# caojiezhang/CiaoSR

Measured on AMD Instinct MI355X. Metric: HR Mpix/s (RDN-CiaoSR x4, LocalImplicitSR forward_test), higher is better.
Workload: dtype f32; 1 GPU; C3: RDN-CiaoSR (c64b16) x4, LR 1356x2040 -> 5424x8160 (DIV2K-shaped 2K LR), tiled inference: 117 tiles of 192x192 (overlap 32), random-init weights, fp32; scale=4, tiles=117, parallelism=tile-shard x1

## Files before the change

### ciaosr_amd/csrc/csa_scores_f32.hip

```cpp
#include "ops.h"

namespace ciaosr {

typedef float f32x16 __attribute__((ext_vector_type(16)));
typedef int i32x4 __attribute__((ext_vector_type(4)));

constexpr int BSH = 8, BSW = 16;
constexpr int BLH = 4, BLW = 16;
constexpr int BHW = BSW + 2;
constexpr int BPN = (BSH + 2) * BHW;
constexpr int BLN = (BLH + 2) * BHW;
constexpr int BDP = 109;
constexpr int BDB = BPN * BDP * 4;
constexpr size_t kBoxLds = 2 * (size_t)BDB;
constexpr unsigned kOobB = 0xFFFFFFF0u;

struct BoxP {
    const float* M; int ldm; unsigned m_bytes; int Hp, Wp;
    int y0, y1;
    const float* R; int ldr; unsigned r_bytes; int Hl, Wl;
    const float* nrm;
    float* S; int lds_; size_t s_floats;
    int pbx, lbx, n_lb, n_items;
};

__global__ void csa_key_norms_kernel(const float* __restrict__ R, int ldr, int Hl, int Wl, int Ch, float floor_, float alpha,
                                     float* __restrict__ nrm) {
    const int lane = threadIdx.x & 63;
    const long l = (long)blockIdx.x * 4 + (threadIdx.x >> 6);
    if (l >= (long)Hl * Wl) return;
    const int ly = (int)(l / Wl), lx = (int)(l - (long)ly * Wl);
    float ss = 0.f;
    for (int e = lane; e < 9 * Ch; e += 64) {
        const int tap = e / Ch, c = e - tap * Ch;
        const int y = ly + tap / 3 - 1, x = lx + tap % 3 - 1;
        if (y >= 0 && y < Hl && x >= 0 && x < Wl) {
            const float v = R[((size_t)y * Wl + x) * ldr + c];
            ss += v * v;
        }
    }
#pragma unroll
    for (int o = 32; o > 0; o >>= 1) ss += __shfl_xor(ss, o, 64);
    if (lane == 0) nrm[l] = alpha / fmaxf(sqrtf(ss), floor_);
}

__global__ __launch_bounds__(512) void csa_scores_box_f32_kernel(BoxP p) {
    extern __shared__ __attribute__((aligned(16))) float Dl[];
    const int t = threadIdx.x, lane = t & 63, wv = __builtin_amdgcn_readfirstlane(t >> 6), li = lane & 31, lh = lane >> 5;
    const int per = (p.n_items + (int)gridDim.x - 1) / (int)gridDim.x;
    const int i0 = (int)blockIdx.x * per, i1 = min(i0 + per, p.n_items);
    if (i0 >= i1) return;
    auto item_pb = [&](int it) -> int { return it / p.n_lb; };
    auto item_lb = [&](int it) -> int { return it - (it / p.n_lb) * p.n_lb; };

    if (wv < 4) {
        const __amdgpu_buffer_rsrc_t rs_m = __builtin_amdgcn_make_buffer_rsrc(const_cast<float*>(p.M), 0, p.m_bytes, 0x00020000);
        const __amdgpu_buffer_rsrc_t rs_r = __builtin_amdgcn_make_buffer_rsrc(const_cast<float*>(p.R), 0, p.r_bytes, 0x00020000);
        auto row_off = [&](int h, int hn, int y0, int x0, int Hh, int Ww, int ld) -> unsigned {
            const int hy = h / BHW, hx = h - hy * BHW;
            const int y = y0 - 1 + hy, x = x0 - 1 + hx;
            return (h < hn && y >= 0 && y < Hh && x >= 0 && x < Ww) ? (unsigned)(((size_t)y * Ww + x) * ld * 4) + (unsigned)lh * 16u : kOobB;
        };
        i32x4 fa[6][4];
        i32x4 fbc[4], fbn[4];
        auto load_a = [&](int pb) {
            const int py0 = p.y0 + (pb / p.pbx) * BSH, px0 = (pb % p.pbx) * BSW;
#pragma unroll
            for (int pt = 0; pt < 6; ++pt) {
                const unsigned mo = row_off(32 * pt + li, BPN, py0, px0, p.Hp, p.Wp, p.ldm);
#pragma unroll
                for (int j = 0; j < 4; ++j) fa[pt][j] = __builtin_amdgcn_raw_buffer_load_b128(rs_m, mo == kOobB ? (int)kOobB : (int)(mo + 32u * j), 0, 0);
            }
        };
        auto load_b = [&](int lb, i32x4 (&f)[4]) {
            const int ly0 = (lb / p.lbx) * BLH, lx0 = (lb % p.lbx) * BLW;
            const unsigned ro = row_off(32 * wv + li, BLN, ly0, lx0, p.Hl, p.Wl, p.ldr);
#pragma unroll
            for (int j = 0; j < 4; ++j) f[j] = __builtin_amdgcn_raw_buffer_load_b128(rs_r, ro == kOobB ? (int)kOobB : (int)(ro + 32u * j), 0, 0);
        };
        int cur_pb = item_pb(i0);
        load_a(cur_pb);
        load_b(item_lb(i0), fbc);
#pragma unroll 1
        for (int it = i0; it <= i1; ++it) {
            if (it < i1) {
                const int k = (it - i0) & 1;
                if (it + 1 < i1) load_b(item_lb(it + 1), fbn);
                float* D = Dl + k * (BDB / 4);
                const int lcol = 32 * wv + li;
#pragma unroll
                for (int pt = 0; pt < 6; ++pt) {
                    f32x16 acc;
#pragma unroll
                    for (int e = 0; e < 16; ++e) acc[e] = 0.f;
#pragma unroll
                    for (int j = 0; j < 4; ++j) {
                        const i32x4 a = fa[pt][j], b = fbc[j];
                        acc = __builtin_amdgcn_mfma_f32_32x32x2f32(__int_as_float(a.x), __int_as_float(b.x), acc, 0, 0, 0);
                        acc = __builtin_amdgcn_mfma_f32_32x32x2f32(__int_as_float(a.y), __int_as_float(b.y), acc, 0, 0, 0);
                        acc = __builtin_amdgcn_mfma_f32_32x32x2f32(__int_as_float(a.z), __int_as_float(b.z), acc, 0, 0, 0);
                        acc = __builtin_amdgcn_mfma_f32_32x32x2f32(__int_as_float(a.w), __int_as_float(b.w), acc, 0, 0, 0);
                    }
                    if (lcol < BLN) {
                        float* dcol = D + (4 * lh) * BDP + lcol;
#pragma unroll
                        for (int r = 0; r < 16; ++r) {
                            constexpr int kLast = BPN - 1;
                            const int rr = 32 * pt + (r & 3) + 8 * (r >> 2);
                            if (rr + 4 <= kLast) dcol[rr * BDP] = acc[r];
                            else if (rr <= kLast && lh == 0) dcol[rr * BDP] = acc[r];
                        }
                    }
                }
#pragma unroll
                for (int j = 0; j < 4; ++j) fbc[j] = fbn[j];
                if (it + 1 < i1 && item_pb(it + 1) != cur_pb) {
                    cur_pb = item_pb(it + 1);
                    load_a(cur_pb);
                }
            }
            __syncthreads();
        }
    } else {
        const int lyy = lane >> 4, lxx = lane & 15;
        int lcol9[9];
#pragma unroll
        for (int a = 0; a < 3; ++a)
#pragma unroll
            for (int b = 0; b < 3; ++b) lcol9[3 * a + b] = (lyy + a) * BHW + lxx + b;
        const int q0 = 32 * (wv - 4);
#pragma unroll 1
        for (int it = i0; it <= i1; ++it) {
            if (it > i0) {
                const int ci = it - 1, k = (ci - i0) & 1;
                const int pb = item_pb(ci), lb = item_lb(ci);
                const int py0 = p.y0 + (pb / p.pbx) * BSH, px0 = (pb % p.pbx) * BSW;
                const int ly = (lb / p.lbx) * BLH + lyy, lx = (lb % p.lbx) * BLW + lxx;
                const bool l_ok = ly < p.Hl && lx < p.Wl;
                const float sc = l_ok ? p.nrm[(size_t)ly * p.Wl + lx] : 0.f;
                const float* D = Dl + k * (BDB / 4) + (q0 >> 4) * BHW * BDP;
                const unsigned lane_off = l_ok ? (unsigned)((size_t)ly * p.Wl + lx) * 4u : kOobB;
                const int qy0 = py0 + (q0 >> 4);
                const size_t s_base = ((size_t)(qy0 - p.y0) * p.Wp + px0) * p.lds_;
                const size_t s_left = p.s_floats > s_base ? (p.s_floats - s_base) * 4 : 0;
                const size_t s_span = ((size_t)p.Wp + BSW) * p.lds_ * 4;
                const __amdgpu_buffer_rsrc_t rs_s =
                    __builtin_amdgcn_make_buffer_rsrc(p.S + s_base, 0, (unsigned)(s_left < s_span ? s_left : s_span), 0x00020000);
                const float* dk[9];
#pragma unroll
                for (int e = 0; e < 9; ++e) dk[e] = D + lcol9[e];
#pragma unroll
                for (int q = 0; q < 32; ++q) {
                    const int pyy = q >> 4, pxx = q & 15;
                    float s = dk[0][(pyy * BHW + pxx) * BDP];
#pragma unroll
                    for (int e = 1; e < 9; ++e) s += dk[e][((pyy + e / 3) * BHW + pxx + e % 3) * BDP];
                    const bool row_ok = qy0 + pyy < p.y1 && px0 + pxx < p.Wp;
                    const unsigned soff = (unsigned)(((size_t)pyy * p.Wp + pxx) * p.lds_ * 4);
                    __builtin_amdgcn_raw_buffer_store_b32(__float_as_int(s * sc), rs_s, (int)(row_ok ? lane_off : kOobB), (int)(row_ok ? soff : 0u), 0);
                }
            }
            __syncthreads();
        }
    }
}

bool csa_scores_box_ok(int Ch, int ldm, int ldr) { return Ch == 32 && (ldm & 3) == 0 && (ldr & 3) == 0; }

int csa_key_norms(const float* R, int ldr, int Hl, int Wl, int Ch, float alpha, float floor_, float* nrm, hipStream_t s) {
    CIAOSR_CHECK_ARG(R && nrm && csa_scores_box_ok(Ch, Ch, ldr));
    ProfScope prof("csa_key_norms", s);
    hipLaunchKernelGGL(csa_key_norms_kernel, dim3(ceil_div((long)Hl * Wl, 4)), dim3(256), 0, s, R, ldr, Hl, Wl, Ch, floor_, alpha, nrm);
    return launch_status("csa_key_norms");
}

int csa_scores_box_f32(const float* M, int ldm, int Hp, int Wp, const float* R, int ldr, int Hl, int Wl, int Ch, const float* nrm, float* S,
                       int ld_s, int y0, int y1, hipStream_t s) {
    CIAOSR_CHECK_ARG(M && R && nrm && S && csa_scores_box_ok(Ch, ldm, ldr) && aligned16(M) && aligned16(R) && 0 <= y0 && y0 < y1 && y1 <= Hp);
    const size_t mb = (size_t)Hp * Wp * ldm * 4, rb = (size_t)Hl * Wl * ldr * 4;
    const size_t s_floats = ((size_t)(y1 - y0) * Wp - 1) * ld_s + (size_t)Hl * Wl;
    CIAOSR_CHECK_ARG(mb < 0xFFFFFF00ull && rb < 0xFFFFFF00ull && ((size_t)Wp + BSW) * ld_s * 4 < 0xFFFFFF00ull);
    BoxP p;
    p.M = M; p.ldm = ldm; p.m_bytes = (unsigned)mb; p.Hp = Hp; p.Wp = Wp; p.y0 = y0; p.y1 = y1;
    p.R = R; p.ldr = ldr; p.r_bytes = (unsigned)rb; p.Hl = Hl; p.Wl = Wl;
    p.nrm = nrm; p.S = S; p.lds_ = ld_s; p.s_floats = s_floats;
    p.pbx = ceil_div(Wp, BSW); p.lbx = ceil_div(Wl, BLW);
    p.n_lb = ceil_div(Hl, BLH) * p.lbx;
    const long n_items = (long)ceil_div(y1 - y0, BSH) * p.pbx * p.n_lb;
    CIAOSR_CHECK_ARG(n_items < 0x7FFFFFFF);
    p.n_items = (int)n_items;
    CIAOSR_BIG_LDS(csa_scores_box_f32_kernel, kBoxLds);
    ProfScope prof("csa_scores", s);
    hipLaunchKernelGGL(csa_scores_box_f32_kernel, dim3(p.n_items < 256 ? p.n_items : 256), dim3(512), kBoxLds, s, p);
    return launch_status("csa_scores_box_f32");
}

}
```

### ciaosr_amd/csrc/csattn.hip

```cpp
#include "ops.h"

namespace ciaosr {

struct CsaPlan {
    int H, W, C, sc, Hp, Wp, HWp, Hl, Wl, L, Lld, Lld8, Ch;
    int band_rows, up, down, s_rows;
    size_t n_V, n_S, n_Y;
    bool banded() const { return band_rows < Hp; }
};

static CsaPlan csa_plan(int H, int W, int C, int sc) {
    CsaPlan p;
    p.H = H; p.W = W; p.C = C; p.sc = sc; p.Ch = (int)round_up(C / 2, 4);
    p.Hp = (int)round_up((size_t)H, sc); p.Wp = (int)round_up((size_t)W, sc);
    p.HWp = p.Hp * p.Wp; p.Hl = p.Hp / sc; p.Wl = p.Wp / sc; p.L = p.Hl * p.Wl;
    p.Lld = (int)round_up(p.L, 4); p.Lld8 = (int)round_up(p.L, 8);
    p.band_rows = p.s_rows = p.Hp; p.up = p.down = 0;
    p.n_V = (size_t)p.L * 9 * sc * sc * C; p.n_S = (size_t)p.HWp * p.Lld; p.n_Y = (size_t)sc * sc * p.HWp * C;
    return p;
}

static bool csa_composed(const CsaPlan& p, const ciaosr_options_t* opt) {
    const int composed_min = opt && opt->csa_composed_min ? opt->csa_composed_min : 4096;
    return p.sc == 2 && composed_min > 0 && p.HWp >= composed_min;
}
static bool csa_wants_four(const CsaPlan& p, Prec prec, const ciaosr_options_t* opt, int s_rows) {
    return prec == kF32 && !(opt && opt->csa_attn_v16) && csa_composed(p, opt) && csa_attn_v4_ok(p.Hp, p.Wp, p.C, p.Lld, s_rows);
}

constexpr int kCsaItemRows = 8;
constexpr int kCsaMinRows16 = 4;
static void csa_plan_bands(CsaPlan& p, Prec prec, const ciaosr_options_t* opt) {
    if (!opt || opt->csa_block_mb <= 0) return;
    const size_t budget = (size_t)opt->csa_block_mb << 20, row_s = (size_t)p.Wp * p.Lld * sizeof(float);
    const size_t row = row_s + (prec != kF32 ? (size_t)p.Wp * p.Lld8 * 2 : 0);
    if (budget >= row * p.Hp) return;
    const size_t min_rows = prec == kF32 ? kCsaItemRows : kCsaMinRows16;
    const bool four = csa_wants_four(p, prec, opt, kCsaItemRows);
    size_t sr = budget / row;
    const size_t addr = ((four ? 0x80000000ull : 0xFFFFFF00ull) - 1) / row_s;
    if (sr > addr) sr = addr;
    if (sr >= 2 * kCsaItemRows) sr -= sr % kCsaItemRows;
    if (sr < min_rows) sr = min_rows;
    const int halo = four ? 3 : 0;
    if (sr >= (size_t)p.Hp + halo) return;
    p.band_rows = (int)sr - halo; p.up = four ? 2 : 0; p.down = four ? 1 : 0;
    p.s_rows = (int)sr < p.Hp ? (int)sr : p.Hp;
    p.n_S = (size_t)p.s_rows * p.Wp * p.Lld;
}

struct CsaBuffers : CsaPlan {
    float *xp, *E, *M, *x2, *R, *Qp, *Kn, *V, *S, *O, *Y, *Yp, *PE, *Pc, *Vp, *Ov, *Er;
    unsigned short* P16;
    float* stats() const { return banded() ? V : Qp; }
    float* norms() const { return Kn; }
    float* partial4() const { return O; }
    float* vedge() const { return Vp; }
    float* edge_rows() const { return banded() ? Er : S; }
    float* splitk() const { return Y; }
    float* softmax_scratch() const { return S; }
    unsigned short* q16() const { return reinterpret_cast<unsigned short*>(Y); }
    unsigned short* k16() const { return q16() + round_up((size_t)HWp * 9 * Ch, 128); }
    unsigned short* vpT() const { return reinterpret_cast<unsigned short*>(V); }
    float* otop() const { return Ov; }
    float* oleft() const { return Ov + (size_t)Wp * 4 * C; }
    float* otl() const { return oleft() + (size_t)Hp * 4 * C; }
};
static bool qk16_fits(const CsaPlan& p) { return ((size_t)p.HWp + p.L) * 9 * p.Ch * 2 + 512 <= p.n_Y * sizeof(float); }
static bool vpt_fits(const CsaPlan& p) { return (size_t)25 * p.C * p.Lld8 * 2 <= p.n_V * sizeof(float); }
static bool softmax16_fits(const CsaPlan& p, const H16Ops& h) { return h.softmax_gemm_scratch((long)p.s_rows * p.Wp, p.L) <= p.n_S; }

template <class Take>
static CsaBuffers csa_carve(const CsaPlan& p, bool p16, Take take) {
    const size_t HW = p.HWp, L = p.L, C = p.C, Ch = p.Ch, n_PE = (size_t)(p.Hp / 2 + 3) * (p.Wp / 2 + 3) * 9 * C;
    CsaBuffers b = {p};
    b.xp = take(HW * C);
    b.E = take(HW * C); b.M = take(HW * Ch);
    b.x2 = take(L * C); b.R = take(L * Ch);
    b.Qp = take(HW * 9 * Ch); b.Kn = take(L * 9 * Ch);
    b.V = take(p.n_V);
    b.S = take(p.n_S);
    b.O = take(HW * 9 * p.sc * p.sc * C);
    b.Y = take(p.n_Y); b.Yp = take((size_t)p.H * p.W * 9 * C);
    b.PE = take(n_PE); b.Pc = take(n_PE);
    b.Vp = take(L * 25 * C);
    b.Ov = take((size_t)(p.Hp + p.Wp) * 4 * C + C);
    b.P16 = reinterpret_cast<unsigned short*>(take((p16 ? (size_t)p.s_rows * p.Wp * p.Lld8 / 2 : 0) + 64));
    b.Er = p.banded() ? take((size_t)(p.Wp + p.Hp) * p.Lld) : nullptr;
    return b;
}
static size_t csa_carve_bytes(const CsaPlan& p, bool p16) {
    size_t n = 0;
    csa_carve(p, p16, [&](size_t floats) { n += floats; return (float*)nullptr; });
    return n * sizeof(float) + 24 * 256;
}

enum CsaScores { kScoresBox, kScoresGemm, kScores16 };
enum CsaTail { kTailUncomposed, kTail16C, kTailFour, kTail16 };
struct CsaRoute {
    CsaScores scores; CsaTail tail;
    bool tile128;
    bool fused_softmax;
};

static CsaRoute csa_route(const CsaPlan& p, Prec prec, const ciaosr_options_t* opt, const ciaosr_csattn_weights_t* w) {
    CsaRoute r = {kScoresGemm, kTailUncomposed, opt && opt->csa_attn_tile128, false};
    if (prec == kF32 && !(opt && opt->csa_scores_gemm) && csa_scores_box_ok(p.Ch, p.Ch, p.Ch)) r.scores = kScoresBox;
    if (!(csa_composed(p, opt) && w->w_down_masked)) return r;
    if (prec != kF32 && (9 * p.Ch) % 8 == 0 && (p.Lld & 3) == 0 && qk16_fits(p) && vpt_fits(p)) {
        r.scores = kScores16; r.tail = kTail16;
        r.fused_softmax = softmax16_fits(p, h16_ops(prec)) && w->softmax_scale > 0.f;
    } else if (csa_wants_four(p, prec, opt, p.s_rows)) {
        r.tail = kTailFour;
    } else {
        r.tail = kTail16C;
    }
    return r;
}
static bool csa_attn_big(const CsaPlan& p, const CsaRoute& r, int M) {
    return !r.tile128 && gemm_big_softmax_f32_ok(p.Lld, 25 * p.C, M, 16 * p.C, p.L, true) &&
           ((size_t)(M - 1) * p.Lld + p.L) * sizeof(float) < 0xFFFFFF00ull;
}

struct CsaBand {
    int y0, y1, ya, yb;
    bool first() const { return y0 == 0; }
};

#define CSA_RUN(x) do { const int rc_ = (x); if (rc_ != CIAOSR_OK) return rc_; } while (0)
struct CsaCall : CsaBuffers {
    const ciaosr_csattn_weights_t* w; float* out; int ld_out; hipStream_t s;

    CsaBand band(int y0) const {
        const int y1 = y0 + band_rows < Hp ? y0 + band_rows : Hp;
        return {y0, y1, y0 > up ? y0 - up : 0, y1 + down < Hp ? y1 + down : Hp};
    }
    static int npix(const CsaBand& b, int Wp_) { return (b.y1 - b.y0) * Wp_; }

    int conv1x1(const float* src, const float* wgt, const float* bias, float slope, float* dst, int n_out, int rows) const {
        if (gemm_small_ok(rows, n_out, C, C, C) && rows <= 4096)
            return gemm_small_f32(src, C, wgt, C, bias, dst, n_out, nullptr, 0, nullptr, 0, rows, n_out, C, CIAOSR_ACT_PRELU, slope, 1.f, s,
                                  "csa_conv1x1");
        return gemm_f32(src, C, wgt, C, false, dst, n_out, bias, rows, n_out, C, 1.f, CIAOSR_ACT_PRELU, slope, s, "csa_conv1x1");
    }

    int embed(const float* feat_hwc, int ld_feat) const {
        CSA_RUN(pad_reflect(feat_hwc, ld_feat, H, W, C, xp, Hp, Wp, s));
        CSA_RUN(conv1x1(xp, w->w_assembly, w->b_assembly, w->slope_assembly, E, C, HWp));
        CSA_RUN(conv1x1(xp, w->w_match1, w->b_match1, w->slope_match1, M, Ch, HWp));
        CSA_RUN(sc == 2 ? avgpool2(xp, Hp, Wp, C, x2, s) : downsample(xp, Hp, Wp, C, sc, x2, s));
        return conv1x1(x2, w->w_match2, w->b_match2, w->slope_match2, R, Ch, L);
    }

    int scores_operands(const CsaRoute& r, Prec prec) const {
        const int Kq = 9 * Ch;
        if (r.scores == kScoresBox) return csa_key_norms(R, Ch, Hl, Wl, Ch, w->softmax_scale, w->escape_nan, norms(), s);
        CSA_RUN(patch_rows(M, Ch, Hp, Wp, Ch, 3, 1, 1, Hp, Wp, Qp, Kq, 0, 0.f, s, "csa_patch_q"));
        CSA_RUN(patch_rows(R, Ch, Hl, Wl, Ch, 3, 1, 1, Hl, Wl, Kn, Kq, 1, w->escape_nan, s, "csa_patch_k"));
        if (r.scores == kScoresGemm) return CIAOSR_OK;
        const H16Ops& h = h16_ops(prec);
        CSA_RUN(h.cast_rows(Qp, Kq, q16(), Kq, HWp, Kq, s));
        return h.cast_rows(Kn, Kq, k16(), Kq, L, Kq, s);
    }
    int scores(const CsaRoute& r, Prec prec, const CsaBand& b) const {
        const int Kq = 9 * Ch, rows = (b.yb - b.ya) * Wp;
        const size_t q0 = (size_t)b.ya * Wp * Kq;
        if (r.scores == kScoresBox) return csa_scores_box_f32(M, Ch, Hp, Wp, R, Ch, Hl, Wl, Ch, norms(), S, Lld, b.ya, b.yb, s);
        if (r.scores == kScoresGemm)
            return gemm_f32(Qp + q0, Kq, Kn, Kq, false, S, Lld, nullptr, rows, L, Kq, w->softmax_scale, CIAOSR_ACT_NONE, 0.f, s, "csa_scores", HWp);
        const H16Ops& h = h16_ops(prec);
        const char* tag = prec == kF16 ? "csa_scores_f16" : "csa_scores_bf16";
        if (r.fused_softmax)
            return h.softmax_gemm_nt(q16() + q0, Kq, k16(), Kq, P16, Lld8, rows, L, Kq, w->softmax_scale, softmax_scratch(), n_S, s, tag, HWp);
        CSA_RUN(h.gemm_nt(q16() + q0, Kq, k16(), Kq, S, Lld, false, rows, L, Kq, w->softmax_scale, s, tag, HWp));
        return h.softmax_rows(S, rows, L, Lld, P16, Lld8, s);
    }

    int patch_down(const float* src, int Hs, int Ws, int stride, int pad, int OH, int OW, float* dst) const {
        return patch_rows(src, C, Hs, Ws, C, 3, stride, pad, OH, OW, dst, 9 * C, 0, 0.f, s, "csa_patch_down");
    }
    int partial_down() const {
        CSA_RUN(patch_down(E, Hp, Wp, 2, 3, Hl + 3, Wl + 3, PE));
        return gemm_f32(PE, 9 * C, w->w_down_masked, 9 * C, false, Pc, 9 * C, nullptr, (Hl + 3) * (Wl + 3), 9 * C, 9 * C, 1.f, CIAOSR_ACT_NONE, 0.f, s,
                        "csa_down_partial");
    }

    int keep_edge_logits(const CsaBand& b) const {
        if (!banded()) return CIAOSR_OK;
        if (b.first()) CSA_RUN(copy_rows(S, Lld, Wp, Lld, edge_rows(), Lld, s, "csa_edge_rows"));
        return copy_rows(S + (size_t)(b.y0 - b.ya) * Wp * Lld, (long)Wp * Lld, b.y1 - b.y0, Lld, edge_rows() + (size_t)(Wp + b.y0) * Lld, Lld, s,
                         "csa_edge_rows");
    }
    int edges(const float* Vc, int ld, int col0, const float* probs) const {
        auto edge = [&](int pix0, int pix_stride, int col, float* dst, int rows, int n) -> int {
            const float* B = Vc + col0 + col;
            if (probs)
                return gemm_f32_splitk(probs + (size_t)pix0 * Lld, Lld, B, ld, true, dst, n, nullptr, rows, n, L, 1.f, CIAOSR_ACT_NONE, 0.f, splitk(),
                                       n_Y, s, "csa_attn_v_edge");
            const float* A = !banded() ? S : edge_rows() + (size_t)pix0 * Lld;
            return gemm_f32_softmax_a(A, banded() ? Lld : pix_stride * Lld, stats(), pix_stride, B, ld, true, dst, n, rows, n, L, splitk(), n_Y, s,
                                      "csa_attn_v_edge");
        };
        CSA_RUN(edge(0, 1, 0, otop(), Wp, 4 * C));
        CSA_RUN(edge(Wp, Wp, 4 * C, oleft(), Hp, 4 * C));
        return edge(0, 1, 8 * C, otl(), 1, C);
    }
    int finish_16c(const float* probs) const {
        CSA_RUN(edges(Vp, 25 * C, 16 * C, probs));
        return csa_gather_out(O, otop(), oleft(), otl(), w->b_down, H, W, Hp, Wp, C, out, ld_out, 16L * C, 4L * C, 4L * C, s);
    }

    int tail_four(const CsaRoute& r, const CsaBand& b) const {
        CSA_RUN(softmax_stats_rows(S, (long)(b.yb - b.ya) * Wp, L, Lld, stats() + 2 * (size_t)b.ya * Wp, s));
        if (b.first()) {
            CSA_RUN(partial_down());
            CSA_RUN(csa_gather_vedge(Pc, Hl, Wl, C, vedge(), s));
        }
        CSA_RUN(csa_attn_v4_f32(S, Lld, stats(), Pc, partial4(), Hp, Wp, C, r.tile128, b.ya, b.yb - b.ya, b.y0, b.y1, s));
        return keep_edge_logits(b);
    }
    int finish_four() const {
        CSA_RUN(edges(vedge(), 9 * C, 0, nullptr));
        return csa_attn_v4_combine(partial4(), otop(), oleft(), otl(), w->b_down, H, W, Hp, Wp, C, out, ld_out, s);
    }

    int tail_16c(const CsaRoute& r, const CsaBand& b) const {
        const int rows = npix(b, Wp);
        float* st = stats() + 2 * (size_t)b.y0 * Wp;
        float* Ob = O + (size_t)b.y0 * Wp * 16 * C;
        CSA_RUN(softmax_stats_rows(S, rows, L, Lld, st, s));
        if (b.first()) {
            CSA_RUN(partial_down());
            CSA_RUN(csa_gather_vprime(Pc, Hl, Wl, C, Vp, s));
        }
        CSA_RUN(csa_attn_big(*this, r, rows) ? gemm_big_softmax_f32(S, Lld, st, 1, Vp, 25 * C, Ob, 16 * C, rows, 16 * C, L, s, "csa_attn_v")
                                             : gemm_f32_softmax_a(S, Lld, st, 1, Vp, 25 * C, true, Ob, 16 * C, rows, 16 * C, L, nullptr, 0, s, "csa_attn_v"));
        return keep_edge_logits(b);
    }

    int tail_16(Prec prec, const CsaBand& b) const {
        const H16Ops& h = h16_ops(prec); const bool f16 = prec == kF16;
        if (b.first()) {
            CSA_RUN(partial_down());
            CSA_RUN(csa_gather_vprime_t_h16(Pc, Hl, Wl, C, vpT(), Lld8, f16, s));
        }
        CSA_RUN(h.gemm_nt(P16, Lld8, vpT(), Lld8, O + (size_t)b.y0 * Wp * 16 * C, 16 * C, false, npix(b, Wp), 16 * C, Lld8, 1.f, s,
                          f16 ? "csa_attn_v_f16" : "csa_attn_v_bf16", HWp));
        if (!banded()) return CIAOSR_OK;
        if (b.first()) CSA_RUN(h.rows_to_f32(P16, Lld8, 0, 1, Wp, Lld, edge_rows(), Lld, s));
        return h.rows_to_f32(P16, Lld8, 0, Wp, b.y1 - b.y0, Lld, edge_rows() + (size_t)(Wp + b.y0) * Lld, Lld, s);
    }
    int finish_16(Prec prec) const {
        const H16Ops& h = h16_ops(prec);
        CSA_RUN(csa_gather_vprime(Pc, Hl, Wl, C, Vp, s));
        if (!banded()) {
            CSA_RUN(h.rows_to_f32(P16, Lld8, 0, 1, Wp, Lld, edge_rows(), Lld, s));
            CSA_RUN(h.rows_to_f32(P16, Lld8, 0, Wp, Hp, Lld, edge_rows() + (size_t)Wp * Lld, Lld, s));
        }
        return finish_16c(edge_rows());
    }

    int tail_uncomposed(const CsaBand& b) const {
        const int kv = 9 * sc * sc * C, rows = npix(b, Wp);
        CSA_RUN(softmax_rows(S, rows, L, Lld, s));
        if (b.first()) CSA_RUN(patch_rows(E, C, Hp, Wp, C, 3 * sc, sc, sc, Hl, Wl, V, kv, 0, 0.f, s, "csa_patch_v"));
        return gemm_f32(S, Lld, V, kv, true, O + (size_t)b.y0 * Wp * kv, kv, nullptr, rows, kv, L, 1.f, CIAOSR_ACT_NONE, 0.f, s, "csa_attn_v", HWp);
    }
    int finish_uncomposed() const {
        const int kv = 9 * sc * sc * C;
        CSA_RUN(sc == 2 ? fold(O, kv, Hp, Wp, C, Y, s) : fold_s(O, kv, Hp, Wp, C, sc, Y, s));
        CSA_RUN(patch_down(Y, sc * Hp, sc * Wp, sc, 1, H, W, Yp));
        if (gemm_small_ok(H * W, C, 9 * C, 9 * C, 9 * C) && H * W <= 4096)
            return gemm_small_f32(Yp, 9 * C, w->w_down, 9 * C, w->b_down, out, ld_out, nullptr, 0, nullptr, 0, H * W, C, 9 * C, CIAOSR_ACT_NONE, 0.f,
                                  1.0f / 6.0f, s, "csa_down");
        return gemm_f32(Yp, 9 * C, w->w_down, 9 * C, false, out, ld_out, w->b_down, H * W, C, 9 * C, 1.0f / 6.0f, CIAOSR_ACT_NONE, 0.f, s, "csa_down");
    }
};

}

using namespace ciaosr;

static int csa_scale(int scale) { return scale < 2 || scale > 4 ? 4 : scale; }

extern "C" size_t ciaosr_cs_attn_workspace_bytes(int H, int W, int C) { return ciaosr_cs_attn_workspace_bytes_scale(H, W, C, 2); }
extern "C" size_t ciaosr_cs_attn_workspace_bytes_scale(int H, int W, int C, int scale) {
    return csa_carve_bytes(csa_plan(H, W, C, csa_scale(scale)), true);
}
extern "C" size_t ciaosr_cs_attn_workspace_bytes_opt(int H, int W, int C, int scale, const ciaosr_options_t* opt) {
    size_t n = 0;
    for (const Prec prec : {kF32, kF16}) {
        CsaPlan p = csa_plan(H, W, C, csa_scale(scale));
        csa_plan_bands(p, prec, opt);
        const size_t m = csa_carve_bytes(p, !p.banded() || prec != kF32);
        n = m > n ? m : n;
    }
    return n;
}
extern "C" int ciaosr_cs_attn_block_rows(int H, int W, int C, int scale, int precision, const ciaosr_options_t* opt) {
    if (H < 1 || W < 1 || C < 1 || scale < 2 || scale > 4 || precision < 0 || precision > 2 || !options_ok(opt)) return 0;
    CsaPlan p = csa_plan(H, W, C, scale);
    csa_plan_bands(p, (Prec)precision, opt);
    return p.band_rows;
}

static int cs_attn(const float* feat_hwc, int ld_feat, int H, int W, const ciaosr_csattn_weights_t* w, float* out, int ld_out,
                   const ciaosr_options_t* opt, void* workspace, size_t workspace_bytes, void* stream, Prec prec) {
    CIAOSR_CHECK_ARG(feat_hwc && w && out && workspace && H >= 2 && W >= 2);
    CIAOSR_CHECK_ARG(options_ok(opt));
    const int C = w->channels, sc = w->scale ? w->scale : 2;
    CIAOSR_CHECK_ARG(C >= 4 && (C & 3) == 0 && ld_feat >= C && (ld_feat & 3) == 0 && (ld_out & 3) == 0);
    CIAOSR_CHECK_ARG(sc >= 2 && sc <= 4 && H >= sc && W >= sc);
    CsaPlan p = csa_plan(H, W, C, sc);
    csa_plan_bands(p, prec, opt);
    const CsaRoute r = csa_route(p, prec, opt, w);
    if (r.tail != kTailFour) p.up = p.down = 0;
    if (workspace_bytes < (p.banded() ? ciaosr_cs_attn_workspace_bytes_opt(H, W, C, sc, opt) : ciaosr_cs_attn_workspace_bytes_scale(H, W, C, sc)))
        return CIAOSR_ERR_WORKSPACE;
    Arena ar(workspace, workspace_bytes);
    const CsaCall c = {csa_carve(p, !p.banded() || prec != kF32, [&](size_t floats) { return ar.take<float>(floats); }), w, out, ld_out,
                       (hipStream_t)stream};
    if (!ar.ok) return CIAOSR_ERR_WORKSPACE;
    CSA_RUN(c.embed(feat_hwc, ld_feat));
    CSA_RUN(c.scores_operands(r, prec));
    for (int y0 = 0; y0 < p.Hp; y0 += p.band_rows) {
        const CsaBand b = c.band(y0);
        CSA_RUN(c.scores(r, prec, b));
        CSA_RUN(r.tail == kTailFour ? c.tail_four(r, b) : r.tail == kTail16C ? c.tail_16c(r, b) : r.tail == kTail16 ? c.tail_16(prec, b)
                                                                                                                   : c.tail_uncomposed(b));
    }
    if (r.tail == kTailFour) return c.finish_four();
    if (r.tail == kTail16C) return c.finish_16c(nullptr);
    if (r.tail == kTail16) return c.finish_16(prec);
    return c.finish_uncomposed();
}

extern "C" int ciaosr_cs_attn_f32(const float* feat_hwc, int ld_feat, int H, int W, const ciaosr_csattn_weights_t* w, float* out, int ld_out,
                                  const ciaosr_options_t* opt, void* workspace, size_t workspace_bytes, void* stream) {
    return cs_attn(feat_hwc, ld_feat, H, W, w, out, ld_out, opt, workspace, workspace_bytes, stream, kF32);
}
extern "C" int ciaosr_cs_attn_bf16(const float* feat_hwc, int ld_feat, int H, int W, const ciaosr_csattn_weights_t* w, float* out, int ld_out,
                                   const ciaosr_options_t* opt, void* workspace, size_t workspace_bytes, void* stream) {
    return cs_attn(feat_hwc, ld_feat, H, W, w, out, ld_out, opt, workspace, workspace_bytes, stream, kBF16);
}
extern "C" int ciaosr_cs_attn_f16(const float* feat_hwc, int ld_feat, int H, int W, const ciaosr_csattn_weights_t* w, float* out, int ld_out,
                                  const ciaosr_options_t* opt, void* workspace, size_t workspace_bytes, void* stream) {
    return cs_attn(feat_hwc, ld_feat, H, W, w, out, ld_out, opt, workspace, workspace_bytes, stream, kF16);
}
```

### ciaosr_amd/csrc/ops.h

```cpp
#pragma once
#include "common.h"

namespace ciaosr {

constexpr int MAXJ = 9;

struct HeadRowsP {
    const float* coord;
    const float* cell;
    long q0;
    int nq, chunk, H, W, local_size, J;
    const float* Tk;
    const float* Tv;
    const float* tailK;
    const float* tailV;
    int ld_tail_k, ld_tail_v;
    int wk0, wv0, relu_k, relu_v;
    float* Hk;
    float* Hv;
    int* q_idx;
    int* k_idx;
};

struct LocalAttnP {
    const float* U;
    int ldu, D, Dv;
    const int* q_idx;
    const int* k_idx;
    const float* wk; int ldwk;
    const float* wv; int ldwv;
    float* z; int ldz;
    int Q, J;
    float scale;
};

struct DecodeP {
    const float* h; int ldh, width;
    const float* w; int ldw;
    const float* b;
    const float* x_lr;
    const float* coord;
    long q0;
    int nq, H, W;
    float* rgb;
};

int gemm_f32(const float* A, int lda, const float* B, int ldb, bool b_kn, float* C, int ldc, const float* bias,
             int M, int N, int K, float alpha, int act, float slope, hipStream_t stream, const char* tag, int plan_rows = 0);
int gemm_f32_splitk(const float* A, int lda, const float* B, int ldb, bool b_kn, float* C, int ldc, const float* bias,
                    int M, int N, int K, float alpha, int act, float slope, float* partial, size_t partial_floats,
                    hipStream_t stream, const char* tag);
int gemm_f32_softmax_a(const float* A, int lda, const float* a_stats2, int a_stats_stride, const float* B, int ldb, bool b_kn, float* C, int ldc,
                       int M, int N, int K, float* partial, size_t partial_floats, hipStream_t stream, const char* tag);
bool gemm_big_softmax_f32_ok(int lda, int ldb, int M, int N, int K, bool b_kn);
int gemm_big_softmax_f32(const float* A, int lda, const float* a_stats2, int a_stats_stride, const float* B, int ldb, float* C, int ldc,
                         int M, int N, int K, hipStream_t stream, const char* tag);
bool gemm_small_ok(int M, int N, int K, int lda, int ldw);
int gemm_small_f32(const float* A, int lda, const float* W, int ldw, const float* bias, float* C, int ldc, float* C2, int ldc2,
                   const float* res, int ldres, int M, int N, int K, int act, float slope, float alpha, hipStream_t s, const char* tag);
int dense_wino_tiles(int H, int W);
int dense_layer_wino_f32(float* X, int ldx, int H, int W, int l, const float* frag_wino, const float* bias, int n_img, hipStream_t s);
int dense_wino4_tiles(int H, int W);
int dense_layer_wino4_f32(float* X, int ldx, int H, int W, int l, const float* frag_wino4, const float* bias, int n_img, hipStream_t s);
int wino_table_f32(const float* Pi, int H, int W, const float* frag_wino, int n_blk, float* out, int ldg, hipStream_t s);
int wino4_table_f32(const float* Pi, int H, int W, const float* frag_wino4, int n_blk, float* out, int ldg, hipStream_t s);
bool csa_scores_box_ok(int Ch, int ldm, int ldr);
int csa_key_norms(const float* R, int ldr, int Hl, int Wl, int Ch, float alpha, float floor_, float* nrm, hipStream_t s);
int csa_scores_box_f32(const float* M, int ldm, int Hp, int Wp, const float* R, int ldr, int Hl, int Wl, int Ch, const float* nrm, float* S,
                       int ld_s, int y0, int y1, hipStream_t s);
bool conv1x1_resident_ok(long M, int N, int K, int ldx, int ldw);
int conv1x1_resident_f32(const float* X, int ldx, const float* W, int ldw, const float* bias, const float* res, int ldres, float* dst,
                         int ld_dst, float* dst2, int ld_dst2, long M, int K, hipStream_t s, const char* tag);
bool conv3x3_small_ok(int H, int W, int Cin, int Cout, int ld_src, int act);
int conv3x3_small(const float* src, int ld_src, int H, int W, int Cin, const float* frag, const float* bias, int Cout, float* dst,
                  int ld_dst, float* dst2, int ld_dst2, const float* res, int ld_res, int act, float alpha, hipStream_t s,
                  const char* tag);
int nchw_to_hwc(const float* src, float* dst, int C, int H, int W, int ld, hipStream_t s);
int hwc_to_nchw(const float* src, int ld, float* dst, int C, int H, int W, hipStream_t s);
int pad_reflect(const float* src, int ld_src, int H, int W, int C, float* dst, int Hp, int Wp, hipStream_t s);
int avgpool2(const float* src, int Hp, int Wp, int C, float* dst, hipStream_t s);
int patch_rows(const float* src, int ld_src, int Hs, int Ws, int Cs, int k, int stride, int pad, int OH, int OW,
               float* out, int ld_out, int normalize, float floor_, hipStream_t s, const char* tag);
int copy_rows(const float* src, long row_stride, int nrows, int cols, float* dst, int ld_dst, hipStream_t s, const char* tag);
int softmax_rows(float* S, long rows, int L, int ld, hipStream_t s);
int softmax_stats_rows(const float* S, long rows, int L, int ld, float* stats2 , hipStream_t s);
int fold(const float* O, int ldo, int Hp, int Wp, int C, float* Y, hipStream_t s);
int fold_s(const float* O, int ldo, int Hp, int Wp, int C, int scale, float* Y, hipStream_t s);
int downsample(const float* src, int Hp, int Wp, int C, int scale, float* dst, hipStream_t s);
int csa_gather_vprime(const float* Pc, int Hh, int Wh, int C, float* Vp, hipStream_t s);
int csa_gather_out(const float* Op, const float* Otop, const float* Oleft, const float* Otl, const float* bd, int H, int W,
                   int Hp, int Wp, int C, float* out, int ld_out, long ld_main, long ld_top, long ld_left, hipStream_t s);
int csa_gather_vprime_t_h16(const float* Pc, int Hh, int Wh, int C, unsigned short* VpT, int ldt, bool f16, hipStream_t s);
bool csa_attn_v4_ok(int Hp, int Wp, int C, int Lld, int s_rows);
int csa_attn_v4_f32(const float* S, int Lld, const float* stats2, const float* Pc, float* part, int Hp, int Wp, int C, bool tile128,
                    int ys, int s_rows, int oy0, int oy1, hipStream_t s);
int csa_gather_vedge(const float* Pc, int Hh, int Wh, int C, float* Ve, hipStream_t s);
int csa_attn_v4_combine(const float* part, const float* Otop, const float* Oleft, const float* Otl, const float* bd, int H, int W, int Hp,
                        int Wp, int C, float* out, int ld_out, hipStream_t s);
int head_indices(const float* coord, const float* cell, long q0, int nq, int chunk, int H, int W, int local_size,
                 int* q_idx, int* k_idx, float* rel, hipStream_t s);
int head_rows(const HeadRowsP& p, hipStream_t s);
int qk_rows(const float* U, int ldu, int D, int H, int W, long row0, int nrows, const float* bias_out, float* A, float* G,
            int ldg, int rows_h16 , hipStream_t s);
int qk_maps(const float* F, int ldf, int C, int H, int W, float* Pi, hipStream_t s);
int transpose_cast_h16(const float* W, int ld, int K, int N, unsigned short* out, bool f16, hipStream_t s);
int local_attention(const LocalAttnP& p, hipStream_t s);
int decode_residual(const DecodeP& p, hipStream_t s);

struct FusedChain {
    const float* table;
    const float* tail;
    int ld_tail;
    const void* frag_hidden[CIAOSR_MAX_LAYERS];
    const void* frag_hidden_lo[CIAOSR_MAX_LAYERS];
    const float* bias_hidden[CIAOSR_MAX_LAYERS];
    int n_hidden;
    const void* frag_out;
    const void* frag_out_lo;
    const float* bias_out;
    int n_out;
};
struct FusedKVP {
    const float* coord;
    const float* cell;
    long q0;
    int nq, chunk, H, W;
    const float* U;
    int ldu, D, Dv;
    unsigned u_bytes;
    FusedChain k, v;
    float softmax_scale;
    float* Z;
    int ldz;
    const float* G;
    int ldg;
    unsigned g_bytes;
    int rows_per_wg;
    const int* gate;
};
struct FusedQP {
    const float* Z; int ldz, Dv;
    const void* frag_in;
    const void* frag_in_lo;
    const float* bias_in;
    int nj_in;
    const void* frag_hidden[CIAOSR_MAX_LAYERS];
    const void* frag_hidden_lo[CIAOSR_MAX_LAYERS];
    const float* bias_hidden[CIAOSR_MAX_LAYERS];
    int n_hidden;
    const float* w_last; int ld_last;
    const float* b_last;
    const float* x_lr;
    const float* coord;
    long q0;
    int nq, H, W;
    float* rgb;
    int rows_per_wg;
};
int head_kv_fused(const FusedKVP& p, hipStream_t s);
int head_decode_fused(const FusedQP& p, hipStream_t s);

#define CIAOSR_H16_DECLS                                                                                                              \
    int gemm_h16_nt(const unsigned short* A, int lda, const unsigned short* B, int ldb, void* C, int ldc, bool c_bf16, int M, int N,  \
                    int K, float alpha, hipStream_t s, const char* tag, int plan_rows );                    \
    int cast_rows_h16(const float* src, int ld_src, unsigned short* dst, int ld_dst, long rows, int cols, hipStream_t s);             \
    int linear_h16(const unsigned short* A, int lda, const unsigned short* W16, int ldw, const float* bias, bool relu, void* C, int ldc,      \
                   bool c_16bit, int M, int N, int K, hipStream_t s, const char* tag);                                                      \
    int softmax_rows_h16(const float* S, long rows, int L, int ld, unsigned short* P, int ldp, hipStream_t s);                        \
    int head_kv_fused_h16(const FusedKVP& p, hipStream_t s);                                                                          \
    int head_decode_fused_h16(const FusedQP& p, hipStream_t s);                                                                       \
    bool head_chain_ok(const ciaosr_head_weights_t* w);                                                                               \
    size_t head_chain_bytes(const ciaosr_head_weights_t* w, int pairs);                                                               \
    int pack_head_chain(const ciaosr_head_weights_t* w, int pairs, void* out, hipStream_t s);                                         \
    bool head_decode_chain_ok(const ciaosr_head_weights_t* w);                                                                        \
    size_t head_kv_chain_bytes(const ciaosr_head_weights_t* w, int pairs);                                                            \
    int head_decode_chain_h16(const FusedQP& qp, const ciaosr_head_weights_t* w, const void* blob, int pairs, hipStream_t s);         \
    int head_kv_chain_h16(const FusedKVP& kp, const ciaosr_head_weights_t* w, const void* blob, int pairs, int grid_w, int* flag,     \
                          hipStream_t s);                                                                                             \
    int pack_fragments_h16(const float* W, int ld, int N, int K, void* P, hipStream_t s, int residual, void* P_lo);                   \
    namespace wide {                                                                                                                  \
    int head_kv_fused_wide(const FusedKVP& p, int mode, hipStream_t s);                                                               \
    int head_decode_fused_wide(const FusedQP& p, int mode, hipStream_t s);                                                            \
    }                                                                                                                                 \
    int dense_h16_tiles(int H, int W);                                                                                                \
    int cast_group_h16(const float* X, int ldx, unsigned short* Xb, int ldxb, int col, long HW, hipStream_t s);                       \
    int dense_layer_h16(float* X, int ldx, unsigned short* Xb, int ldxb, int H, int W, int l, const void* frag16,                     \
                        const void* frag16_lo, const float* bias, int n_img, hipStream_t s, int route);                               \
    int conv1x1_h16(const unsigned short* A, int lda, const unsigned short* W16, int ldw, const float* bias, const float* res,        \
                    int ldres, float* out, int ldo, float* out2, int ldo2, unsigned short* out16, int ldo16, int M, int N, int K,     \
                    hipStream_t s, const char* tag);                                                                                  \
    int cast_many_h16(const float* const* src, int n, int rows, int cols, unsigned short* dst, hipStream_t s);                       \
    size_t softmax_gemm_scratch_floats(long M, int N);                                                                                \
    int softmax_gemm_h16_nt(const unsigned short* A, int lda, const unsigned short* B, int ldb, unsigned short* P, int ldp, int M,    \
                            int N, int K, float alpha, float* scratch, size_t scratch_floats, hipStream_t s, const char* tag,         \
                            int plan_rows);                                                                                           \
    int rows_to_f32_h16(const unsigned short* src, long ld_src, long row0, long row_stride, int nrows, int cols, float* dst,          \
                        int ld_dst, hipStream_t s);
namespace b16 { CIAOSR_H16_DECLS }
namespace f16 { CIAOSR_H16_DECLS }
#undef CIAOSR_H16_DECLS


enum Prec { kF32 = 0, kBF16 = 1, kF16 = 2 };

struct Mode {
    Prec trunk;
    bool trunk_pairs;
    bool lff16;
    bool lo;
    bool x3;
    bool hoist16;
    bool table16;
};
inline Mode resolve_mode(Prec entry, const ciaosr_options_t* opt) {
    const int pairs = entry == kF32 || !opt ? 0 : opt->f16_pairs;
    const bool single = entry == kBF16 && opt && opt->bf16_single;
    Mode m;
    m.x3 = pairs == 2 || (entry == kF16 && pairs == 3);
    m.lo = (entry == kBF16 && (!single || m.x3)) || (entry == kF16 && pairs != 0);
    m.trunk = pairs == 2 ? kF32 : entry;
    m.trunk_pairs = m.trunk != kF32 && m.lo;
    m.lff16 = m.trunk == kF16 && !m.trunk_pairs;
// ... 60 lines not shown
```

Before: 11.98 Mpix/s.

## Fuse online softmax statistics into box score kernel, merge partials per pixel

The CSA box score kernel now computes running max and sum-of-exp per query pixel while it writes scores. Each row-chunk's partials are reduced across lanes with butterfly shuffles and stored, then a small merge kernel combines them into final softmax stats. This replaces the separate softmax_stats_rows pass that re-read the whole score matrix. The consumer side also moves to 8 waves with 16 queries each, and LDS reads are software-pipelined. Work is split across blocks in whole key-row chunks. The cost is more consumer register pressure and an extra scratch buffer that aliases Y.

```diff
diff --git a/ciaosr_amd/csrc/csa_scores_f32.hip b/ciaosr_amd/csrc/csa_scores_f32.hip
--- a/ciaosr_amd/csrc/csa_scores_f32.hip
+++ b/ciaosr_amd/csrc/csa_scores_f32.hip
@@ -15,6 +15,13 @@
 constexpr size_t kBoxLds = 2 * (size_t)BDB;
 constexpr unsigned kOobB = 0xFFFFFFF0u;
 
+#ifdef CIAOSR_PROBE
+__device__ unsigned long long g_boxprobe[256 * 16];
+#define BOXPROBE_T() __builtin_readcyclecounter()
+#else
+#define BOXPROBE_T() 0ull
+#endif
+
 struct BoxP {
     const float* M; int ldm; unsigned m_bytes; int Hp, Wp;
     int y0, y1;
@@ -22,7 +29,22 @@
     const float* nrm;
     float* S; int lds_; size_t s_floats;
     int pbx, lbx, n_lb, n_items;
+    int n_chunks;
+    float2* part; size_t part_ld;
 };
+
+constexpr float kLog2eS = 1.4426950408889634f;
+constexpr int NCW = 8;
+constexpr int NQ = BSH * BSW / NCW;
+constexpr int QG = 4;
+constexpr int kBoxThreads = 256 + 64 * NCW;
+static_assert(NQ == 16 && NQ % (2 * QG) == 0, "consumer cut: the chunk-end butterfly is written for 16 outputs per lane");
+
+__device__ __forceinline__ void stat_merge(float& m, float& s, float m2, float s2) {
+    const float mx = fmaxf(m, m2), ref = mx == -INFINITY ? 0.f : mx;
+    s = s * __builtin_amdgcn_exp2f(m - ref) + s2 * __builtin_amdgcn_exp2f(m2 - ref);
+    m = mx;
+}
 
 __global__ void csa_key_norms_kernel(const float* __restrict__ R, int ldr, int Hl, int Wl, int Ch, float floor_, float alpha,
                                      float* __restrict__ nrm) {
@@ -44,12 +66,25 @@
     if (lane == 0) nrm[l] = alpha / fmaxf(sqrtf(ss), floor_);
 }
 
-__global__ __launch_bounds__(512) void csa_scores_box_f32_kernel(BoxP p) {
+template <bool STATS>
+__global__ __launch_bounds__(kBoxThreads) void csa_scores_box_f32_kernel(BoxP p) {
     extern __shared__ __attribute__((aligned(16))) float Dl[];
     const int t = threadIdx.x, lane = t & 63, wv = __builtin_amdgcn_readfirstlane(t >> 6), li = lane & 31, lh = lane >> 5;
-    const int per = (p.n_items + (int)gridDim.x - 1) / (int)gridDim.x;
-    const int i0 = (int)blockIdx.x * per, i1 = min(i0 + per, p.n_items);
-    if (i0 >= i1) return;
+    const int per = (p.n_chunks + (int)gridDim.x - 1) / (int)gridDim.x;
+    const long r0 = (long)blockIdx.x * per * p.lbx;
+    if (r0 >= p.n_items) return;
+    const int i0 = (int)r0, i1 = (int)(r0 + (long)per * p.lbx < p.n_items ? r0 + (long)per * p.lbx : p.n_items);
+#ifdef CIAOSR_PROBE
+    const bool stamp = lane == 0 && (wv == 0 || wv == 4);
+    unsigned long long pacc[6] = {0, 0, 0, 0, 0, 0}, pt0 = BOXPROBE_T();
+    const unsigned long long pstart = pt0;
+#define BOXPROBE_ADD(slot) do { const unsigned long long now_ = BOXPROBE_T(); pacc[slot] += now_ - pt0; pt0 = now_; } while (0)
+#define BOXPROBE_OUT(role) do { if (stamp) { for (int i_ = 0; i_ < 6; ++i_) g_boxprobe[blockIdx.x * 16 + 8 * (role) + i_] = pacc[i_];         \
+        g_boxprobe[blockIdx.x * 16 + 8 * (role) + 6] = BOXPROBE_T() - pstart; g_boxprobe[blockIdx.x * 16 + 8 * (role) + 7] = (unsigned long long)(i1 - i0); } } while (0)
+#else
+#define BOXPROBE_ADD(slot) do { } while (0)
+#define BOXPROBE_OUT(role) do { } while (0)
+#endif
     auto item_pb = [&](int it) -> int { return it / p.n_lb; };
     auto item_lb = [&](int it) -> int { return it - (it / p.n_lb) * p.n_lb; };
 
@@ -85,9 +120,11 @@
         for (int it = i0; it <= i1; ++it) {
             if (it < i1) {
                 const int k = (it - i0) & 1;
+                BOXPROBE_ADD(0);
                 if (it + 1 < i1) load_b(item_lb(it + 1), fbn);
                 float* D = Dl + k * (BDB / 4);
                 const int lcol = 32 * wv + li;
+                BOXPROBE_ADD(1);
 #pragma unroll
                 for (int pt = 0; pt < 6; ++pt) {
                     f32x16 acc;
@@ -101,6 +138,7 @@
                         acc = __builtin_amdgcn_mfma_f32_32x32x2f32(__int_as_float(a.z), __int_as_float(b.z), acc, 0, 0, 0);
                         acc = __builtin_amdgcn_mfma_f32_32x32x2f32(__int_as_float(a.w), __int_as_float(b.w), acc, 0, 0, 0);
                     }
+                    BOXPROBE_ADD(2);
                     if (lcol < BLN) {
                         float* dcol = D + (4 * lh) * BDP + lcol;
 #pragma unroll
@@ -111,6 +149,7 @@
                             else if (rr <= kLast && lh == 0) dcol[rr * BDP] = acc[r];
                         }
                     }
+                    BOXPROBE_ADD(3);
                 }
 #pragma unroll
                 for (int j = 0; j < 4; ++j) fbc[j] = fbn[j];
@@ -118,9 +157,12 @@
                     cur_pb = item_pb(it + 1);
                     load_a(cur_pb);
                 }
+                BOXPROBE_ADD(4);
             }
             __syncthreads();
+            BOXPROBE_ADD(5);
         }
+        BOXPROBE_OUT(0);
     } else {
         const int lyy = lane >> 4, lxx = lane & 15;
         int lcol9[9];
@@ -128,7 +170,10 @@
         for (int a = 0; a < 3; ++a)
 #pragma unroll
             for (int b = 0; b < 3; ++b) lcol9[3 * a + b] = (lyy + a) * BHW + lxx + b;
-        const int q0 = 32 * (wv - 4);
+        const int q0 = NQ * (wv - 4);
+        float rm[NQ], rs[NQ];
+#pragma unroll
+        for (int q = 0; q < NQ; ++q) { rm[q] = -INFINITY; rs[q] = 0.f; }
 #pragma unroll 1
         for (int it = i0; it <= i1; ++it) {
             if (it > i0) {
@@ -143,25 +188,83 @@
                 const int qy0 = py0 + (q0 >> 4);
                 const size_t s_base = ((size_t)(qy0 - p.y0) * p.Wp + px0) * p.lds_;
                 const size_t s_left = p.s_floats > s_base ? (p.s_floats - s_base) * 4 : 0;
-                const size_t s_span = ((size_t)p.Wp + BSW) * p.lds_ * 4;
+                const size_t s_span = ((size_t)(NQ / 16 - 1) * p.Wp + BSW) * p.lds_ * 4;
                 const __amdgpu_buffer_rsrc_t rs_s =
                     __builtin_amdgcn_make_buffer_rsrc(p.S + s_base, 0, (unsigned)(s_left < s_span ? s_left : s_span), 0x00020000);
+                BOXPROBE_ADD(0);
                 const float* dk[9];
 #pragma unroll
                 for (int e = 0; e < 9; ++e) dk[e] = D + lcol9[e];
-#pragma unroll
-                for (int q = 0; q < 32; ++q) {
-                    const int pyy = q >> 4, pxx = q & 15;
-                    float s = dk[0][(pyy * BHW + pxx) * BDP];
-#pragma unroll
-                    for (int e = 1; e < 9; ++e) s += dk[e][((pyy + e / 3) * BHW + pxx + e % 3) * BDP];
-                    const bool row_ok = qy0 + pyy < p.y1 && px0 + pxx < p.Wp;
-                    const unsigned soff = (unsigned)(((size_t)pyy * p.Wp + pxx) * p.lds_ * 4);
-                    __builtin_amdgcn_raw_buffer_store_b32(__float_as_int(s * sc), rs_s, (int)(row_ok ? lane_off : kOobB), (int)(row_ok ? soff : 0u), 0);
+                auto read_group = [&](int g, float (&dv)[QG][9]) {
+#pragma unroll
+                    for (int i = 0; i < QG; ++i) {
+                        const int q = QG * g + i, pyy = q >> 4, pxx = q & 15;
+#pragma unroll
+                        for (int e = 0; e < 9; ++e) dv[i][e] = dk[e][((pyy + e / 3) * BHW + pxx + e % 3) * BDP];
+                    }
+                };
+                auto emit_group = [&](int g, const float (&dv)[QG][9]) {
+#pragma unroll
+                    for (int i = 0; i < QG; ++i) {
+                        const int q = QG * g + i, pyy = q >> 4, pxx = q & 15;
+                        float s = dv[i][0];
+#pragma unroll
+                        for (int e = 1; e < 9; ++e) s += dv[i][e];
+                        const bool row_ok = qy0 + pyy < p.y1 && px0 + pxx < p.Wp;
+                        const unsigned soff = (unsigned)(((size_t)pyy * p.Wp + pxx) * p.lds_ * 4);
+                        const float v = s * sc;
+                        __builtin_amdgcn_raw_buffer_store_b32(__float_as_int(v), rs_s, (int)(row_ok ? lane_off : kOobB), (int)(row_ok ? soff : 0u), 0);
+                        if (STATS) {
+                            const float x = v * kLog2eS, d = __builtin_fmaf(v, kLog2eS, -rm[q]);
+                            const float e = __builtin_amdgcn_exp2f(-__builtin_fabsf(d));
+                            const bool up = l_ok && d > 0.f;
+                            rs[q] = up ? __builtin_fmaf(rs[q], e, 1.f) : rs[q] + (l_ok ? e : 0.f);
+                            rm[q] = up ? x : rm[q];
+                        }
+                    }
+                };
+                float da[QG][9], db[QG][9];
+                read_group(0, da);
+#pragma unroll
+                for (int g = 0; g < NQ / QG; g += 2) {
+                    read_group(g + 1, db);
+                    __builtin_amdgcn_sched_barrier(0);
+                    emit_group(g, da);
+                    __builtin_amdgcn_sched_barrier(0);
+                    if (g + 2 < NQ / QG) read_group(g + 2, da);
+                    __builtin_amdgcn_sched_barrier(0);
+                    emit_group(g + 1, db);
+                    __builtin_amdgcn_sched_barrier(0);
                 }
+                BOXPROBE_ADD(1);
+                if (STATS && lb % p.lbx == p.lbx - 1) {
+#define CSA_STAT_STEP(H)                                                                                          \
+    {                                                                                                             \
+        const bool hi = (lane & (LB * (H))) != 0;                                                                 \
+        _Pragma("unroll") for (int j = 0; j < (H); ++j) {                                                         \
+            const float sm = hi ? rm[j] : rm[j + (H)], ss = hi ? rs[j] : rs[j + (H)];                             \
+            float km = hi ? rm[j + (H)] : rm[j], ks = hi ? rs[j + (H)] : rs[j];                                   \
+            stat_merge(km, ks, __shfl_xor(sm, LB * (H), 64), __shfl_xor(ss, LB * (H), 64));                       \
+            rm[j] = km; rs[j] = ks;                                                                               \
+        }                                                                                                         \
+    }
+                    constexpr int LB = 64 / NQ;
+                    CSA_STAT_STEP(8) CSA_STAT_STEP(4) CSA_STAT_STEP(2) CSA_STAT_STEP(1)
+#undef CSA_STAT_STEP
+#pragma unroll
+                    for (int o = LB / 2; o >= 1; o >>= 1) stat_merge(rm[0], rs[0], __shfl_xor(rm[0], o, 64), __shfl_xor(rs[0], o, 64));
+                    const int q = lane / LB, wy = qy0 + (q >> 4), wx = px0 + (q & 15);
+                    if ((lane & (LB - 1)) == 0 && wy < p.y1 && wx < p.Wp)
+                        p.part[(size_t)(lb / p.lbx) * p.part_ld + (size_t)wy * p.Wp + wx] = make_float2(rm[0], rs[0]);
+#pragma unroll
+                    for (int q2 = 0; q2 < NQ; ++q2) { rm[q2] = -INFINITY; rs[q2] = 0.f; }
+                }
+                BOXPROBE_ADD(2);
             }
             __syncthreads();
+            BOXPROBE_ADD(3);
         }
+        BOXPROBE_OUT(1);
     }
 }
 
@@ -174,9 +277,12 @@
     return launch_status("csa_key_norms");
 }
 
+size_t csa_scores_stat_floats(int Hp, int Wp, int Hl) { return (size_t)ceil_div(Hl, BLH) * Hp * Wp * 2; }
+
 int csa_scores_box_f32(const float* M, int ldm, int Hp, int Wp, const float* R, int ldr, int Hl, int Wl, int Ch, const float* nrm, float* S,
-                       int ld_s, int y0, int y1, hipStream_t s) {
+                       int ld_s, int y0, int y1, float* stat_parts, hipStream_t s) {
     CIAOSR_CHECK_ARG(M && R && nrm && S && csa_scores_box_ok(Ch, ldm, ldr) && aligned16(M) && aligned16(R) && 0 <= y0 && y0 < y1 && y1 <= Hp);
+    CIAOSR_CHECK_ARG(!stat_parts || (reinterpret_cast<uintptr_t>(stat_parts) & 7u) == 0);
     const size_t mb = (size_t)Hp * Wp * ldm * 4, rb = (size_t)Hl * Wl * ldr * 4;
     const size_t s_floats = ((size_t)(y1 - y0) * Wp - 1) * ld_s + (size_t)Hl * Wl;
     CIAOSR_CHECK_ARG(mb < 0xFFFFFF00ull && rb < 0xFFFFFF00ull && ((size_t)Wp + BSW) * ld_s * 4 < 0xFFFFFF00ull);
@@ -188,11 +294,48 @@
     p.n_lb = ceil_div(Hl, BLH) * p.lbx;
     const long n_items = (long)ceil_div(y1 - y0, BSH) * p.pbx * p.n_lb;
     CIAOSR_CHECK_ARG(n_items < 0x7FFFFFFF);
-    p.n_items = (int)n_items;
-    CIAOSR_BIG_LDS(csa_scores_box_f32_kernel, kBoxLds);
+    p.n_items = (int)n_items; p.n_chunks = p.n_items / p.lbx;
+    p.part = reinterpret_cast<float2*>(stat_parts); p.part_ld = (size_t)Hp * Wp;
+    const dim3 grid(p.n_chunks < 256 ? p.n_chunks : 256);
     ProfScope prof("csa_scores", s);
-    hipLaunchKernelGGL(csa_scores_box_f32_kernel, dim3(p.n_items < 256 ? p.n_items : 256), dim3(512), kBoxLds, s, p);
+    if (stat_parts) {
+        CIAOSR_BIG_LDS(csa_scores_box_f32_kernel<true>, kBoxLds);
+        hipLaunchKernelGGL(csa_scores_box_f32_kernel<true>, grid, dim3(kBoxThreads), kBoxLds, s, p);
+    } else {
+        CIAOSR_BIG_LDS(csa_scores_box_f32_kernel<false>, kBoxLds);
+        hipLaunchKernelGGL(csa_scores_box_f32_kernel<false>, grid, dim3(kBoxThreads), kBoxLds, s, p);
+    }
     return launch_status("csa_scores_box_f32");
 }
 
-}
+__global__ __launch_bounds__(256) void csa_stats_merge_kernel(const float2* __restrict__ part, size_t part_ld, int n_part, long pix0, long n_pix,
+                                                              float2* __restrict__ stats) {
+    const long i = (long)blockIdx.x * 256 + threadIdx.x;
+    if (i >= n_pix) return;
+    const float2* pr = part + pix0 + i;
+    float m = -INFINITY;
+    for (int c = 0; c < n_part; ++c) m = fmaxf(m, pr[(size_t)c * part_ld].x);
+    float sum = 0.f;
+    for (int c = 0; c < n_part; ++c) {
+        const float2 v = pr[(size_t)c * part_ld];
+        sum += v.y * __builtin_amdgcn_exp2f(v.x - m);
+    }
+    stats[pix0 + i] = make_float2(m, 1.f / sum);
+}
+
+int csa_scores_stats_merge(const float* stat_parts, int Hp, int Wp, int Hl, int y0, int y1, float* stats2, hipStream_t s) {
+    CIAOSR_CHECK_ARG(stat_parts && stats2 && 0 <= y0 && y0 < y1 && y1 <= Hp);
+    const long n_pix = (long)(y1 - y0) * Wp;
+    ProfScope prof("softmax_stats", s);
+    hipLaunchKernelGGL(csa_stats_merge_kernel, dim3(ceil_div(n_pix, 256)), dim3(256), 0, s, reinterpret_cast<const float2*>(stat_parts),
+                       (size_t)Hp * Wp, ceil_div(Hl, BLH), (long)y0 * Wp, n_pix, reinterpret_cast<float2*>(stats2));
+    return launch_status("csa_scores_stats_merge");
+}
+
+}
+
+#ifdef CIAOSR_PROBE
+extern "C" int ciaosr_debug_probe_box_read(unsigned long long* host, int n_words) {
+    return hipMemcpyFromSymbol(host, HIP_SYMBOL(ciaosr::g_boxprobe), (size_t)n_words * 8) == hipSuccess ? 0 : -1;
+}
+#endif
diff --git a/ciaosr_amd/csrc/csattn.hip b/ciaosr_amd/csrc/csattn.hip
--- a/ciaosr_amd/csrc/csattn.hip
+++ b/ciaosr_amd/csrc/csattn.hip
@@ -58,6 +58,7 @@
     float* vedge() const { return Vp; }
     float* edge_rows() const { return banded() ? Er : S; }
     float* splitk() const { return Y; }
+    float* stat_parts() const { return Y; }
     float* softmax_scratch() const { return S; }
     unsigned short* q16() const { return reinterpret_cast<unsigned short*>(Y); }
     unsigned short* k16() const { return q16() + round_up((size_t)HWp * 9 * Ch, 128); }
@@ -68,6 +69,7 @@
 };
 static bool qk16_fits(const CsaPlan& p) { return ((size_t)p.HWp + p.L) * 9 * p.Ch * 2 + 512 <= p.n_Y * sizeof(float); }
 static bool vpt_fits(const CsaPlan& p) { return (size_t)25 * p.C * p.Lld8 * 2 <= p.n_V * sizeof(float); }
+static bool stat_parts_fits(const CsaPlan& p) { return csa_scores_stat_floats(p.Hp, p.Wp, p.Hl) <= p.n_Y; }
 static bool softmax16_fits(const CsaPlan& p, const H16Ops& h) { return h.softmax_gemm_scratch((long)p.s_rows * p.Wp, p.L) <= p.n_S; }
 
 template <class Take>
@@ -101,10 +103,11 @@
     CsaScores scores; CsaTail tail;
     bool tile128;
     bool fused_softmax;
+    bool box_stats;
 };
 
 static CsaRoute csa_route(const CsaPlan& p, Prec prec, const ciaosr_options_t* opt, const ciaosr_csattn_weights_t* w) {
-    CsaRoute r = {kScoresGemm, kTailUncomposed, opt && opt->csa_attn_tile128, false};
+    CsaRoute r = {kScoresGemm, kTailUncomposed, opt && opt->csa_attn_tile128, false, false};
     if (prec == kF32 && !(opt && opt->csa_scores_gemm) && csa_scores_box_ok(p.Ch, p.Ch, p.Ch)) r.scores = kScoresBox;
     if (!(csa_composed(p, opt) && w->w_down_masked)) return r;
     if (prec != kF32 && (9 * p.Ch) % 8 == 0 && (p.Lld & 3) == 0 && qk16_fits(p) && vpt_fits(p)) {
@@ -115,6 +118,7 @@
     } else {
         r.tail = kTail16C;
     }
+    r.box_stats = r.scores == kScoresBox && r.tail != kTail16 && stat_parts_fits(p);
     return r;
 }
 static bool csa_attn_big(const CsaPlan& p, const CsaRoute& r, int M) {
@@ -165,7 +169,8 @@
     int scores(const CsaRoute& r, Prec prec, const CsaBand& b) const {
         const int Kq = 9 * Ch, rows = (b.yb - b.ya) * Wp;
         const size_t q0 = (size_t)b.ya * Wp * Kq;
-        if (r.scores == kScoresBox) return csa_scores_box_f32(M, Ch, Hp, Wp, R, Ch, Hl, Wl, Ch, norms(), S, Lld, b.ya, b.yb, s);
+        if (r.scores == kScoresBox)
+            return csa_scores_box_f32(M, Ch, Hp, Wp, R, Ch, Hl, Wl, Ch, norms(), S, Lld, b.ya, b.yb, r.box_stats ? stat_parts() : nullptr, s);
         if (r.scores == kScoresGemm)
             return gemm_f32(Qp + q0, Kq, Kn, Kq, false, S, Lld, nullptr, rows, L, Kq, w->softmax_scale, CIAOSR_ACT_NONE, 0.f, s, "csa_scores", HWp);
         const H16Ops& h = h16_ops(prec);
@@ -210,8 +215,13 @@
         return csa_gather_out(O, otop(), oleft(), otl(), w->b_down, H, W, Hp, Wp, C, out, ld_out, 16L * C, 4L * C, 4L * C, s);
     }
 
+    int row_stats(const CsaRoute& r, int ya, int yb) const {
+        if (r.box_stats) return csa_scores_stats_merge(stat_parts(), Hp, Wp, Hl, ya, yb, stats(), s);
+        return softmax_stats_rows(S, (long)(yb - ya) * Wp, L, Lld, stats() + 2 * (size_t)ya * Wp, s);
+    }
+
     int tail_four(const CsaRoute& r, const CsaBand& b) const {
-        CSA_RUN(softmax_stats_rows(S, (long)(b.yb - b.ya) * Wp, L, Lld, stats() + 2 * (size_t)b.ya * Wp, s));
+        CSA_RUN(row_stats(r, b.ya, b.yb));
         if (b.first()) {
             CSA_RUN(partial_down());
             CSA_RUN(csa_gather_vedge(Pc, Hl, Wl, C, vedge(), s));
@@ -228,7 +238,7 @@
         const int rows = npix(b, Wp);
         float* st = stats() + 2 * (size_t)b.y0 * Wp;
         float* Ob = O + (size_t)b.y0 * Wp * 16 * C;
-        CSA_RUN(softmax_stats_rows(S, rows, L, Lld, st, s));
+        CSA_RUN(row_stats(r, b.y0, b.y1));
         if (b.first()) {
             CSA_RUN(partial_down());
             CSA_RUN(csa_gather_vprime(Pc, Hl, Wl, C, Vp, s));
diff --git a/ciaosr_amd/csrc/ops.h b/ciaosr_amd/csrc/ops.h
--- a/ciaosr_amd/csrc/ops.h
+++ b/ciaosr_amd/csrc/ops.h
@@ -67,7 +67,9 @@
 bool csa_scores_box_ok(int Ch, int ldm, int ldr);
 int csa_key_norms(const float* R, int ldr, int Hl, int Wl, int Ch, float alpha, float floor_, float* nrm, hipStream_t s);
 int csa_scores_box_f32(const float* M, int ldm, int Hp, int Wp, const float* R, int ldr, int Hl, int Wl, int Ch, const float* nrm, float* S,
-                       int ld_s, int y0, int y1, hipStream_t s);
+                       int ld_s, int y0, int y1, float* stat_parts, hipStream_t s);
+size_t csa_scores_stat_floats(int Hp, int Wp, int Hl);
+int csa_scores_stats_merge(const float* stat_parts, int Hp, int Wp, int Hl, int y0, int y1, float* stats2, hipStream_t s);
 bool conv1x1_resident_ok(long M, int N, int K, int ldx, int ldw);
 int conv1x1_resident_f32(const float* X, int ldx, const float* W, int ldw, const float* bias, const float* res, int ldres, float* dst,
                          int ld_dst, float* dst2, int ld_dst2, long M, int K, hipStream_t s, const char* tag);
```

After: 12.10 Mpix/s (median of 6 runs). No clear change (+1.0%).
